# sflorescu/BWA-MEM_GPU

Hardware: AMD Instinct MI355X
Metric: Mreads/s (150 bp single-end vs hg38-scale index; seed-and-extend hot path) (higher is better)
Workload: dtype u16

## Files before the change

bwa-mem_gpu_amd/csrc/seed_kernels.hip:

```cpp
#include <cstring>
#include <string>
#include <vector>
#include <hip/hip_runtime.h>
#include <rocprim/rocprim.hpp>
#include <stdint.h>
#include <stdio.h>
#include <stdlib.h>
#include "bmh_internal.h"
#include "wtrace.h"
#include "fmd_dev.h"
#include "seed_dev.h"


__device__ __forceinline__ int ascii_code(uint8_t ch)
{
	ch &= 0xDF;
	return ch == 'A' ? 0 : ch == 'C' ? 1 : ch == 'G' ? 2 : ch == 'T' ? 3 : 4;
}

#define PACK_READS_PER_BLOCK 64
__global__ void __launch_bounds__(256) pack_reads_kernel(const uint8_t *__restrict__ ascii, const uint32_t *__restrict__ offs,
                                                         const uint32_t *__restrict__ lens, uint32_t n_reads, uint32_t n_grp,
                                                         uint32_t lds_bytes, uint32_t *__restrict__ pk, uint32_t *__restrict__ nm)
{
	wtrace_scope_t wt_(WT_PACK);
	extern __shared__ __attribute__((aligned(16))) uint8_t stage[];
	const uint32_t r0 = blockIdx.x * PACK_READS_PER_BLOCK;
	const uint32_t nr = min((uint32_t)PACK_READS_PER_BLOCK, n_reads - r0);
	const uint32_t first = offs[r0], last = offs[r0 + nr - 1] + lens[r0 + nr - 1];
	const uint32_t abase = first & ~3u;
	const bool staged = last >= first && (last - abase) + 4 <= lds_bytes && (((uintptr_t)ascii) & 3) == 0;
	if (staged) {
		const uint32_t nw = (last - abase + 3) >> 2;
		const uint32_t *src = (const uint32_t *)(ascii + abase);
		for (uint32_t i = threadIdx.x; i < nw; i += blockDim.x) ((uint32_t *)stage)[i] = src[i];
	}
	__syncthreads();
	for (uint32_t it = threadIdx.x; it < nr * n_grp; it += blockDim.x) {
		const uint32_t rr = it % nr, g = it / nr, r = r0 + rr;
		const uint32_t len = lens[r], o = offs[r];
		const bool in_lds = staged && o >= first && o + len <= last;
		const uint8_t *p = in_lds ? stage + (o - abase) : ascii + o;
		uint32_t w0 = 0, w1 = 0, m = 0;
		for (int t = 0; t < 32; ++t) {
			const uint32_t i = g * 32 + t;
			const int c = i < len ? ascii_code(p[i]) : 4;
			if (c > 3) m |= 1u << t;
			else if (t < 16) w0 |= (uint32_t)c << (2 * t);
			else w1 |= (uint32_t)c << (2 * (t - 16));
		}
		pk[(size_t)(2 * g) * n_reads + r] = w0;
		pk[(size_t)(2 * g + 1) * n_reads + r] = w1;
		nm[(size_t)g * n_reads + r] = m;
	}
}


struct cand_t { uint32_t read, xe, j, s; };

#define CAND_CHUNK 1024u
#define CAND_INVALID 0xFFFFFFFFu
// ... 126 lines not shown
		cand_append(want, c, ck, out_a, out_k, counter, cap, cc);
	}
	cand_fill_invalid(cc, out_a, cap);
	if (live) n_cand[r] = j;
	if (iters_out && live) iters_out[r] = it_mine;
	if (fst) {
		if (live) { atomicAdd(fst + 1, (unsigned long long)it_mine); atomicAdd(fst + 8 + (it_mine / 8u < 31u ? it_mine / 8u : 31u), 1ull); }
		if ((threadIdx.x & 63) == 0) { atomicAdd(fst, (unsigned long long)it_wave); atomicAdd(fst + 2, 1ull); atomicMax(fst + 3, (unsigned long long)it_wave); atomicAdd(fst + 40 + (it_wave / 8u < 23u ? it_wave / 8u : 23u), 1ull); }
	}
}


__global__ void __launch_bounds__(256) cand_scatter_kernel(const cand_t *__restrict__ in_a, uint64_t n_list, const uint32_t *__restrict__ cand_base,
                                                           uint32_t *__restrict__ perm)
{
	uint64_t t = (uint64_t)blockIdx.x * blockDim.x + threadIdx.x;
	if (t >= n_list) return;
	const uint2 h = *(const uint2 *)&in_a[t];
	const uint32_t j = in_a[t].j;
	if (h.x == CAND_INVALID) return;
	perm[(size_t)cand_base[h.x] + j] = (uint32_t)t;
}

__global__ void __launch_bounds__(256) iota_kernel(uint32_t *__restrict__ v, uint32_t n) { const uint32_t i = blockIdx.x * 256u + threadIdx.x; if (i < n) v[i] = i; }
#define BWD_NSUB 64
struct bwd_state_t { uint64_t lo, hi; uint32_t read, t; uint16_t x, end, i, beg; };
template <bool RESUME>
__global__ void __launch_bounds__(256) smem_backward_kernel(fmd_dev_t f, read_view_t rv, uint64_t n_cands, int min_seed_len,
                                                            const cand_t *__restrict__ cand_a, const uint64_t *__restrict__ cand_k,
                                                            const uint32_t *__restrict__ perm,
                                                            res_t *__restrict__ res_a, uint64_t *__restrict__ res_k,
                                                            unsigned long long *__restrict__ stats,
                                                            const bwd_state_t *__restrict__ in_state, const uint32_t *__restrict__ in_count,
                                                            bwd_state_t *__restrict__ out_state, uint32_t *__restrict__ out_count, const uint32_t sub_cap, const int max_iter)
{
	wtrace_scope_t wt_(WT_BACKWARD);
	fmd_wave_prio(f.wave_prio);
	uint64_t t = (uint64_t)blockIdx.x * blockDim.x + threadIdx.x;
	const int lane = __lane_id();
	__shared__ uint64_t l2_lds[4];
	if (threadIdx.x < 4) l2_lds[threadIdx.x] = f.L2[threadIdx.x];
	__syncthreads();
	const uint32_t sub = blockIdx.x % BWD_NSUB;
	if (RESUME) {
		n_cands = in_count[sub];
		t = (uint64_t)(blockIdx.x / BWD_NSUB) * blockDim.x + threadIdx.x;
		in_state += (size_t)sub * sub_cap;
		if ((uint64_t)(blockIdx.x / BWD_NSUB) * blockDim.x >= n_cands) return;
	}
	if (out_state) { out_state += (size_t)sub * sub_cap; out_count += sub; }
	bool live = t < n_cands;
	cand_t c = {CAND_INVALID, 0, 0, 0};
	uint64_t lo = 0, hi = 0;
	int x = 0, end = 0, i = -1, beg = 0;
	uint32_t t_out = (uint32_t)t;
	if (RESUME) {
		if (live) { const bwd_state_t s = in_state[t]; lo = s.lo; hi = s.hi; c.read = s.read; t_out = s.t; x = s.x; end = s.end; i = s.i; beg = s.beg; c.s = (uint32_t)(hi - lo + 1); }
	} else {
		if (live) { const uint32_t src = perm[t]; c = cand_a[src]; lo = cand_k[src]; hi = lo + c.s - 1; }
		x = (int)(c.xe >> 16); end = (int)(c.xe & 0xFFFF);
		i = x - 1; beg = x;
	}
	bool act = live && i >= 0, dropped = false;
	const uint32_t nread = __shfl_down(c.read, 1), nx = __shfl_down((uint32_t)x, 1), nt = __shfl_down(t_out, 1);
	const bool last_of_seg = lane == 63 || !live || nread != c.read || nx != (uint32_t)x || nt <= t_out;
	const unsigned long long segb = __ballot(last_of_seg);
	const int seg_end = lane + __builtin_ctzll(segb >> lane);
// ... 13 lines not shown
			const uint64_t L2b = l2_lds[b];
			const uint64_t nl = L2b + ol + 1, nu = L2b + ou;
			const bool ok = !isn && nl <= nu;
			lo = ok ? nl : lo; hi = ok ? nu : hi; beg = ok ? i : beg;
			size = ok ? (uint32_t)(nu - nl + 1) : size;
			i -= ok ? 1 : 0;
			act = ok && i >= 0;
			if (act && (i & 15) == 15) {
				rw = rv.pk[(size_t)(i >> 4) * rv.n_reads + c.read];
				if ((i & 31) == 31) rm = rv.nm[(size_t)(i >> 5) * rv.n_reads + c.read];
			}
		}
		const unsigned long long am = __ballot(act) & above;
		const int nxt = am ? __builtin_ctzll(am) : lane;
		const uint32_t nsize = __shfl(size, nxt);
		if (act && am && nsize == size) { act = false; dropped = true; }
	}
	if (stats) {
		if (live && !RESUME) atomicAdd(stats + 8 + (st_mine < 39u ? st_mine : 39u), 1ull);
		atomicAdd(stats + 1, (unsigned long long)st_steps); atomicAdd(stats + 4, (unsigned long long)st_uniq); atomicAdd(stats + 5, (unsigned long long)st_u0); atomicAdd(stats + 6, (unsigned long long)st_x0); { const bool nowalk = !__any(live && !st_x0); if (!RESUME && lane == 0 && nowalk) atomicAdd(stats + 7, 1ull); }
		if (lane == 0) { atomicAdd(stats, (unsigned long long)st_iter); atomicAdd(stats + 2, 1ull); atomicMax(stats + 3, (unsigned long long)st_iter); }
	}
	const unsigned long long sm = __ballot(act);
	if (sm) {
		const int first = (int)__builtin_ctzll(sm);
		uint32_t base = 0;
		if (lane == first) base = atomicAdd(out_count, (uint32_t)__builtin_popcountll(sm));
		base = __shfl(base, first);
		if (act) {
			bwd_state_t s; s.lo = lo; s.hi = hi; s.read = c.read; s.t = t_out; s.x = (uint16_t)x; s.end = (uint16_t)end; s.i = (uint16_t)i; s.beg = (uint16_t)beg;
			out_state[base + (uint32_t)__builtin_popcountll(sm & ((1ull << lane) - 1ull))] = s;
		}
	}
	if (live && !act) {
		res_t o;
		o.read = c.read; o.be = ((uint32_t)beg << 16) | (uint32_t)end;
		o.s = (!dropped && end - beg >= min_seed_len) ? (uint32_t)(hi - lo + 1) : 0u;
		o.pad = 0;
		res_a[t_out] = o;
		res_k[t_out] = lo;
	}
}


__global__ void __launch_bounds__(256) smem_filter_kernel(const res_t *__restrict__ res_a, uint64_t n, uint32_t *__restrict__ occ)
{
	wtrace_scope_t wt_(WT_FILTER);
	uint64_t t = (uint64_t)blockIdx.x * blockDim.x + threadIdx.x;
	res_t e = {0xFFFFFFFEu, 0, 0, 0};
	if (t < n) e = res_a[t];
	bool k = e.s > 0;
	__shared__ uint32_t fv_has[4], fv_read[4], fv_be[4];
	const int lane = __lane_id(), wv = (int)(threadIdx.x >> 6);
	const unsigned long long vm = __ballot(k);
	if (lane == 0) fv_has[wv] = vm ? 1u : 0u;
	if (vm && lane == (int)__builtin_ctzll(vm)) { fv_read[wv] = e.read; fv_be[wv] = e.be; }
	__syncthreads();
	const unsigned long long ab = lane < 63 ? (vm >> (lane + 1)) << (lane + 1) : 0ull;
	const int nl = ab ? __builtin_ctzll(ab) : lane;
	const uint32_t nread = __shfl(e.read, nl), nbe = __shfl(e.be, nl);
	if (k) {
		if (ab) { if (nread == e.read && (nbe >> 16) == (e.be >> 16)) k = false; }
		else {
			int w2 = wv + 1;
			while (w2 < 4 && !fv_has[w2]) ++w2;
			if (w2 < 4) { if (fv_read[w2] == e.read && (fv_be[w2] >> 16) == (e.be >> 16)) k = false; }
			else {
				for (uint64_t u = (uint64_t)(blockIdx.x + 1) * blockDim.x; u < n; ++u) {
					res_t nx = res_a[u];
					if (nx.read != e.read) break;
					if (nx.s == 0) continue;
					if ((nx.be >> 16) == (e.be >> 16)) k = false;
					break;
				}
			}
		}
	}
	if (t <= n) occ[t] = k ? e.s : 0u;
}

struct occ_keep_in {
	const uint32_t *occ;
	__device__ uint64_t operator()(uint64_t t) const { const uint32_t v = occ[t]; return (uint64_t)v | ((uint64_t)(v != 0u) << OCC_OFF_SHIFT); }
};
__global__ void __launch_bounds__(256) per_read_counts_kernel(const uint32_t *__restrict__ cand_base, const uint64_t *__restrict__ occ_off,
                                                              uint32_t n_reads, uint32_t *__restrict__ n_ref_pos, uint32_t *__restrict__ prefix)
{
	uint32_t r = blockIdx.x * blockDim.x + threadIdx.x;
	if (r >= n_reads) return;
	uint64_t a = occ_off[cand_base[r]] & OCC_OFF_MASK, b = occ_off[cand_base[r + 1]] & OCC_OFF_MASK;
	prefix[r] = (uint32_t)a;
	n_ref_pos[r] = (uint32_t)(b - a);
}


__global__ void __launch_bounds__(256) expand_kernel(const res_t *__restrict__ res_a, const uint64_t *__restrict__ res_k,
                                                     const uint32_t *__restrict__ occ, const uint64_t *__restrict__ occ_off, uint64_t n,
                                                     uint64_t *__restrict__ rows, int2 *__restrict__ qbeg, uint32_t *__restrict__ score)
{
	wtrace_scope_t wt_(WT_EXPAND);
	uint64_t t = (uint64_t)blockIdx.x * blockDim.x + threadIdx.x;
	uint32_t s = 0;
	uint64_t k = 0, off = 0;
	int2 qb = make_int2(0, 0);
	if (t < n) {
		s = occ[t];
		if (s) { res_t e = res_a[t]; k = res_k[t]; off = occ_off[t] & OCC_OFF_MASK; qb = make_int2((int)(e.be >> 16), (int)(e.be & 0xFFFF)); }
	}
	const uint32_t SMALL = 4;
	if (s && s <= SMALL) {
		for (uint32_t u = 0; u < s; ++u) { rows[off + u] = k + u; qbeg[off + u] = qb; score[off + u] = u ? 0u : s; }
// ... 205 lines not shown
	uint64_t t = (uint64_t)blockIdx.x * blockDim.x + threadIdx.x;
	bool v = false;
	if (t < n_list) {
		cand_t c = in_a[t];
		v = c.read != CAND_INVALID;
		keys[t] = v ? (((uint64_t)c.read << 16) | (c.xe & 0xFFFFu)) : ~0ull;
		vals[t] = (uint32_t)t;
	}
	unsigned long long m = __ballot(v);
	if (__lane_id() == 0 && m) atomicAdd(n_valid, (unsigned long long)__popcll(m));
}

__global__ void __launch_bounds__(256) smem_gather_kernel(const cand_t *__restrict__ in_a, const uint64_t *__restrict__ in_k,
                                                          const uint32_t *__restrict__ vals, uint64_t n_valid, res_t *__restrict__ res_a,
                                                          uint64_t *__restrict__ res_k, uint32_t *__restrict__ occ)
{
	uint64_t t = (uint64_t)blockIdx.x * blockDim.x + threadIdx.x;
	if (t > n_valid) return;
	if (t == n_valid) { occ[t] = 0; return; }
	const uint32_t src = vals[t];
	const cand_t c = in_a[src];
	res_t o = {c.read, c.xe, c.s, 0};
	res_a[t] = o;
	res_k[t] = in_k[src];
	occ[t] = c.s;
}


#define HIPCK(x) do { hipError_t e_ = (x); if (e_ != hipSuccess) { bmh_set_error("%s: %s", #x, hipGetErrorString(e_)); return BMH_ENODEV; } } while (0)

struct bmh_seed_ws {
	uint32_t max_reads; uint64_t max_bases, max_cands, max_occ;
	uint32_t *pk, *nm;
	uint32_t n_grp_cap;
	cand_t *cand_a; uint64_t *cand_k;
	res_t *res_a; uint64_t *res_k;
	uint32_t *n_cand, *cand_base;
	uint32_t *occ;
	uint64_t *occ_off;
	uint64_t *rows; int2 *qbeg; uint32_t *score;
	uint32_t *n_ref_pos, *prefix;
	unsigned long long *counter;
	uint4 *scratch; size_t scratch_entries;
	uint64_t *skeys, *skeys2; uint32_t *svals, *svals2;
	bwd_state_t *bwd_state[2]; uint64_t bwd_state_cap;
	uint32_t *bwd_cnt;
	uint32_t *fwd_iters; uint32_t fwd_iters_n;
	void *scan_tmp; size_t scan_tmp_bytes;
	hipEvent_t ev[8];
	float ms[7];
	hipStream_t st_hi; hipEvent_t ev_in, ev_out;
	reseed_state_t *rs;
};

extern "C" bmh_seed_ws_t *bmh_seed_ws_create(uint32_t max_reads, uint64_t max_bases, uint64_t max_cands, uint64_t max_occ)
{
	if (max_reads == 0 || max_bases == 0) { bmh_set_error("bmh_seed_ws_create: empty capacity"); return nullptr; }
	bmh_seed_ws *w = (bmh_seed_ws *)calloc(1, sizeof(bmh_seed_ws));
	w->max_reads = max_reads; w->max_bases = max_bases;
	w->max_cands = max_cands ? max_cands : (uint64_t)max_reads * 16 + max_bases * 2 / 5;
	w->max_cands += ((uint64_t)max_reads / 64 + 1) * (CAND_CHUNK + 64);
	w->max_occ = max_occ ? max_occ : (uint64_t)max_reads * 64;
	w->n_grp_cap = 0;
	bool ok = true;
#define A(p, n) ok = ok && hipMalloc((void **)&(p), (size_t)(n)) == hipSuccess
	A(w->cand_a, sizeof(cand_t) * w->max_cands); A(w->cand_k, 8 * w->max_cands);
	A(w->res_a, sizeof(res_t) * (w->max_cands + 1)); A(w->res_k, 8 * (w->max_cands + 1));
	A(w->n_cand, 4 * ((size_t)max_reads + 1)); A(w->cand_base, 4 * ((size_t)max_reads + 1));
	A(w->occ, 4 * (w->max_cands + 1));
	A(w->occ_off, 8 * (w->max_cands + 1));
	A(w->rows, 8 * w->max_occ); A(w->qbeg, 8 * w->max_occ); A(w->score, 4 * w->max_occ);
	A(w->n_ref_pos, 4 * (size_t)max_reads); A(w->prefix, 4 * (size_t)max_reads);
	A(w->counter, 1024);
	A(w->bwd_cnt, 4 * 8 * BWD_NSUB);
	A(w->skeys, 8 * w->max_cands); A(w->skeys2, 8 * w->max_cands); A(w->svals, 4 * w->max_cands); A(w->svals2, 4 * w->max_cands);
	size_t t1 = 0, t2 = 0, t3 = 0;
	rocprim::radix_sort_pairs(nullptr, t3, w->skeys, w->skeys2, w->svals, w->svals2, (size_t)w->max_cands, 0, 64, 0);
	rocprim::exclusive_scan(nullptr, t1, w->n_cand, w->cand_base, 0u, (size_t)max_reads + 1, rocprim::plus<uint32_t>(), 0);
	rocprim::exclusive_scan(nullptr, t2, w->occ, w->occ_off, (uint64_t)0, w->max_cands + 1, rocprim::plus<uint64_t>(), 0);
	w->scan_tmp_bytes = t1 > t2 ? t1 : t2;
	if (t3 > w->scan_tmp_bytes) w->scan_tmp_bytes = t3;
	A(w->scan_tmp, w->scan_tmp_bytes + 256);
#undef A
	for (int i = 0; i < 8; ++i) ok = ok && hipEventCreate(&w->ev[i]) == hipSuccess;
	{
		const char *pe = getenv("BMH_SEED_PRIO");
		if (!(pe && pe[0] == 'n')) {
			int prio_lo = 0, prio_hi = 0;
			(void)hipDeviceGetStreamPriorityRange(&prio_lo, &prio_hi);
			const char *cue = getenv("BMH_SEED_CUS");
			const int n_cus = cue ? atoi(cue) : 0;
			if (n_cus > 0 && n_cus < 256) {
				uint32_t cumask[8] = {0, 0, 0, 0, 0, 0, 0, 0};
				for (int i = 0; i < n_cus; ++i) { const int b = (i * 167 + 13) & 255; cumask[b >> 5] |= 1u << (b & 31); }
				ok = ok && hipExtStreamCreateWithCUMask(&w->st_hi, 8, cumask) == hipSuccess;
			} else
			ok = ok && hipStreamCreateWithPriority(&w->st_hi, hipStreamNonBlocking, prio_hi) == hipSuccess;
			ok = ok && hipEventCreateWithFlags(&w->ev_in, hipEventDisableTiming) == hipSuccess && hipEventCreateWithFlags(&w->ev_out, hipEventDisableTiming) == hipSuccess;
		}
	}
	if (!ok) { bmh_set_error("bmh_seed_ws_create: hipMalloc failed (%s)", hipGetErrorString(hipGetLastError())); bmh_seed_ws_free(w); return nullptr; }
	return w;
}

extern "C" void bmh_seed_ws_free(bmh_seed_ws_t *w)
{
	if (!w) return;
	void *ps[] = {w->pk, w->nm, w->cand_a, w->cand_k, w->res_a, w->res_k, w->n_cand, w->cand_base, w->occ,
	              w->occ_off, w->rows, w->qbeg, w->score, w->n_ref_pos, w->prefix, w->counter, w->scan_tmp,
	              w->scratch, w->skeys, w->skeys2, w->svals, w->svals2, w->bwd_state[0], w->bwd_state[1], w->bwd_cnt, w->fwd_iters};
	for (void *p : ps) if (p) (void)hipFree(p);
	for (int i = 0; i < 8; ++i) if (w->ev[i]) (void)hipEventDestroy(w->ev[i]);
	if (w->st_hi) (void)hipStreamDestroy(w->st_hi);
	if (w->ev_in) (void)hipEventDestroy(w->ev_in);
	if (w->ev_out) (void)hipEventDestroy(w->ev_out);
	reseed_state_free(w->rs);
	free(w);
}

extern "C" void bmh_seed_last_timing(const bmh_seed_ws_t *w, float ms[7]) { memcpy(ms, w->ms, sizeof(float) * 7); }

static inline unsigned nblk(uint64_t n, unsigned b) { return (unsigned)((n + b - 1) / b); }

static int bwd_state_reserve(bmh_seed_ws *w, uint64_t n)
{
	if (n <= w->bwd_state_cap) return BMH_OK;
	for (int k = 0; k < 2; ++k) { if (w->bwd_state[k]) (void)hipFree(w->bwd_state[k]); w->bwd_state[k] = nullptr; }
	w->bwd_state_cap = 0;
	const uint64_t cap = n + n / 8 + 1024;
	for (int k = 0; k < 2; ++k)
		if (hipMalloc((void **)&w->bwd_state[k], sizeof(bwd_state_t) * cap) != hipSuccess) { bmh_set_error("bmh_seed_batch: no memory for %llu parked walks of the backward search", (unsigned long long)cap); return BMH_ENOMEM; }
	w->bwd_state_cap = cap;
	return BMH_OK;
}

static int grow_occ(bmh_seed_ws *w, uint64_t need, bmh_seeds_t *out)
{
	if (need <= w->max_occ) return BMH_OK;
	(void)hipFree(w->rows); (void)hipFree(w->qbeg); (void)hipFree(w->score);
	w->rows = nullptr; w->qbeg = nullptr; w->score = nullptr; w->max_occ = 0;
	const uint64_t cap = need + need / 4 + 1024;
	if (hipMalloc((void **)&w->rows, 8 * cap) != hipSuccess || hipMalloc((void **)&w->qbeg, 8 * cap) != hipSuccess || hipMalloc((void **)&w->score, 4 * cap) != hipSuccess) {
		bmh_set_error("bmh_seed_batch: %llu occurrences: no memory for the output arrays (%s)", (unsigned long long)need, hipGetErrorString(hipGetLastError()));
		return BMH_ECAPACITY;
	}
	w->max_occ = cap;
	out->d_rbeg = w->rows; out->d_qbeg = (const int32_t *)w->qbeg; out->d_score = w->score;
	return BMH_OK;
}

static int seed_batch_on(bmh_seed_ws_t *w, const bmh_index_t *idx, const uint8_t *d_reads, const uint32_t *d_offs,
                         const uint32_t *d_lens, uint32_t n_reads, int min_seed_len, void *stream_, bmh_seeds_t *out, const bmh_reseed_opt_t *ro = nullptr);
static int seed_batch_impl(bmh_seed_ws_t *w, const bmh_index_t *idx, const uint8_t *d_reads, const uint32_t *d_offs,
                           const uint32_t *d_lens, uint32_t n_reads, int min_seed_len, const bmh_reseed_opt_t *ro, void *stream_, bmh_seeds_t *out);
extern "C" int bmh_seed_batch(bmh_seed_ws_t *w, const bmh_index_t *idx, const uint8_t *d_reads, const uint32_t *d_offs,
                              const uint32_t *d_lens, uint32_t n_reads, int min_seed_len, void *stream_, bmh_seeds_t *out)
{
	return seed_batch_impl(w, idx, d_reads, d_offs, d_lens, n_reads, min_seed_len, nullptr, stream_, out);
}
extern "C" void bmh_reseed_opt_default(bmh_reseed_opt_t *o)
{
	if (!o) return;
	o->enable = 0; o->split_factor = 1.5f; o->split_width = 10; o->max_mem_intv = 20;
}
extern "C" int bmh_seed_batch_reseed(bmh_seed_ws_t *w, const bmh_index_t *idx, const uint8_t *d_reads, const uint32_t *d_offs,
                                     const uint32_t *d_lens, uint32_t n_reads, int min_seed_len, const bmh_reseed_opt_t *opt, void *stream_, bmh_seeds_t *out)
{
	return seed_batch_impl(w, idx, d_reads, d_offs, d_lens, n_reads, min_seed_len, (opt && opt->enable) ? opt : nullptr, stream_, out);
}
static int seed_batch_impl(bmh_seed_ws_t *w, const bmh_index_t *idx, const uint8_t *d_reads, const uint32_t *d_offs,
                           const uint32_t *d_lens, uint32_t n_reads, int min_seed_len, const bmh_reseed_opt_t *ro, void *stream_, bmh_seeds_t *out)
{
	if (!w || !idx || !out) { bmh_set_error("bmh_seed_batch: null argument"); return BMH_EINVAL; }
	if (!w->st_hi) return seed_batch_on(w, idx, d_reads, d_offs, d_lens, n_reads, min_seed_len, stream_, out, ro);
	hipStream_t su = (hipStream_t)stream_;
	HIPCK(hipStreamSynchronize(su));
	const int rc = seed_batch_on(w, idx, d_reads, d_offs, d_lens, n_reads, min_seed_len, (void *)w->st_hi, out, ro);
	HIPCK(hipEventRecord(w->ev_out, w->st_hi));
	HIPCK(hipStreamWaitEvent(su, w->ev_out, 0));
	return rc;
}
static int seed_batch_on(bmh_seed_ws_t *w, const bmh_index_t *idx, const uint8_t *d_reads, const uint32_t *d_offs,
                         const uint32_t *d_lens, uint32_t n_reads, int min_seed_len, void *stream_, bmh_seeds_t *out, const bmh_reseed_opt_t *ro)
{
	memset(out, 0, sizeof(*out));
	if (n_reads > w->max_reads) { bmh_set_error("bmh_seed_batch: %u reads > workspace capacity %u", n_reads, w->max_reads); return BMH_ECAPACITY; }
	if (min_seed_len < 1) { bmh_set_error("bmh_seed_batch: min_seed_len < 1"); return BMH_EINVAL; }
	hipStream_t st = (hipStream_t)stream_;
	out->d_rbeg = w->rows; out->d_qbeg = (const int32_t *)w->qbeg; out->d_score = w->score;
	out->d_n_ref_pos = w->n_ref_pos; out->d_prefix = w->prefix;
	memset(w->ms, 0, sizeof(w->ms));
	if (n_reads == 0) return BMH_OK;
	fmd_dev_t f = idx->dev;
	f.wave_prio = bmh_tune("SEED_SETPRIO", 0);
	const unsigned lds_pad = (unsigned)bmh_tune("SEED_LDS_PAD", 0);
	uint32_t max_len = 0;
	{
		uint32_t *d_max = (uint32_t *)w->counter + 2;
		size_t tb = w->scan_tmp_bytes;
		HIPCK(rocprim::reduce(w->scan_tmp, tb, d_lens, d_max, 0u, (size_t)n_reads, rocprim::maximum<uint32_t>(), st));
		HIPCK(hipMemcpyAsync(&max_len, d_max, 4, hipMemcpyDeviceToHost, st));
		HIPCK(hipStreamSynchronize(st));
	}
	if (max_len > 65535) { bmh_set_error("bmh_seed_batch: read longer than 65535 bases"); return BMH_EINVAL; }
	uint32_t n_grp = (max_len + 31) / 32;
	if (n_grp == 0) n_grp = 1;
	if (n_grp > w->n_grp_cap) {
		if (w->pk) (void)hipFree(w->pk);
		if (w->nm) (void)hipFree(w->nm);
		w->pk = w->nm = nullptr; w->n_grp_cap = 0;
		HIPCK(hipMalloc((void **)&w->pk, (size_t)8 * n_grp * w->max_reads));
		HIPCK(hipMalloc((void **)&w->nm, (size_t)4 * n_grp * w->max_reads));
		w->n_grp_cap = n_grp;
	}
	read_view_t rv = {w->pk, w->nm, n_reads};

	HIPCK(hipEventRecord(w->ev[0], st));
	{
		const uint32_t lds_bytes = PACK_READS_PER_BLOCK * n_grp * 32 + 64;
		pack_reads_kernel<<<nblk(n_reads, PACK_READS_PER_BLOCK), 256, lds_bytes <= 65536 ? lds_bytes : 0, st>>>(d_reads, d_offs, d_lens, n_reads, n_grp, lds_bytes <= 65536 ? lds_bytes : 0, w->pk, w->nm);
	}
	static const bool use_fused = getenv("BMH_SEED_FUSED") != nullptr;
	if (use_fused && !ro) {
		const uint32_t depth = max_len >= (uint32_t)min_seed_len ? max_len - (uint32_t)min_seed_len + 1 : 1;
		static int blocks_per_cu = 0, n_cu = 0;
		if (!blocks_per_cu) {
			int dev = 0; hipDeviceProp_t prop;
			HIPCK(hipGetDevice(&dev)); HIPCK(hipGetDeviceProperties(&prop, dev));
			n_cu = prop.multiProcessorCount;
			HIPCK(hipOccupancyMaxActiveBlocksPerMultiprocessor(&blocks_per_cu, smem_fused_kernel, 256, 0));
			if (blocks_per_cu < 1) blocks_per_cu = 1;
		}
		unsigned grid = (unsigned)(n_cu * blocks_per_cu);
		if (grid > nblk(n_reads, 256)) grid = nblk(n_reads, 256);
		const size_t want = (size_t)depth * grid * 256;
		if (want > w->scratch_entries) {
			if (w->scratch) (void)hipFree(w->scratch);
			w->scratch = nullptr; w->scratch_entries = 0;
			HIPCK(hipMalloc((void **)&w->scratch, want * sizeof(uint4)));
			w->scratch_entries = want;
		}
		HIPCK(hipEventRecord(w->ev[1], st));
		HIPCK(hipMemsetAsync(w->counter, 0, 64, st));
		smem_fused_kernel<<<grid, 256, 0, st>>>(f, rv, d_lens, min_seed_len, w->scratch, w->cand_a, w->cand_k, w->counter,
		                                        w->max_cands, w->n_ref_pos, w->counter + 1, (unsigned int *)(w->counter + 3));
		HIPCK(hipEventRecord(w->ev[2], st));
		unsigned long long cnt[8] = {0};
		HIPCK(hipMemcpyAsync(cnt, w->counter, 64, hipMemcpyDeviceToHost, st));
		HIPCK(hipStreamSynchronize(st));
		const unsigned long long n_list = cnt[0];
		out->n_cands = cnt[1];
		if (getenv("BMH_SEED_STATS")) fprintf(stderr, "[fused] grid %u blocks, waves %llu, wave-iterations %llu (%.0f per wave), rank requests %llu (%.1f per iteration), cands %llu\n", grid, cnt[6], cnt[4], (double)cnt[4] / (double)(cnt[6] ? cnt[6] : 1), cnt[5], (double)cnt[5] / (double)(cnt[4] ? cnt[4] : 1), cnt[1]);
		if (n_list > w->max_cands) { bmh_set_error("bmh_seed_batch: %llu SMEM slots > capacity %llu", n_list, (unsigned long long)w->max_cands); return BMH_ECAPACITY; }
		unsigned long long n_valid = 0;
		if (n_list) {
			smem_key_kernel<<<nblk(n_list, 256), 256, 0, st>>>(w->cand_a, n_list, w->skeys, w->svals, w->counter + 2);
			size_t tb = w->scan_tmp_bytes;
			HIPCK(rocprim::radix_sort_pairs(w->scan_tmp, tb, w->skeys, w->skeys2, w->svals, w->svals2, (size_t)n_list, 0, 64, st));
			HIPCK(hipMemcpyAsync(&n_valid, w->counter + 2, 8, hipMemcpyDeviceToHost, st));
			HIPCK(hipStreamSynchronize(st));
		}
		HIPCK(hipEventRecord(w->ev[3], st));
		smem_gather_kernel<<<nblk(n_valid + 1, 256), 256, 0, st>>>(w->cand_a, w->cand_k, w->svals2, n_valid, w->res_a, w->res_k, w->occ);
		{
			size_t tb = w->scan_tmp_bytes;
			HIPCK(rocprim::exclusive_scan(w->scan_tmp, tb, w->occ, w->occ_off, (uint64_t)0, (size_t)n_valid + 1, rocprim::plus<uint64_t>(), st));
			tb = w->scan_tmp_bytes;
			HIPCK(rocprim::exclusive_scan(w->scan_tmp, tb, w->n_ref_pos, w->prefix, 0u, (size_t)n_reads, rocprim::plus<uint32_t>(), st));
		}
		uint64_t tot = 0;
		HIPCK(hipMemcpyAsync(&tot, w->occ_off + n_valid, 8, hipMemcpyDeviceToHost, st));
		HIPCK(hipStreamSynchronize(st));
		out->n_seeds = tot; out->n_smems = n_valid;
		if (grow_occ(w, tot, out) != BMH_OK) return BMH_ECAPACITY;
		if (tot >> 32) { bmh_set_error("bmh_seed_batch: more than 2^32 occurrences in one batch"); return BMH_ECAPACITY; }
		HIPCK(hipEventRecord(w->ev[4], st));
		if (n_valid)
			expand_kernel<<<nblk(n_valid, 256), 256, 0, st>>>(w->res_a, w->res_k, w->occ, w->occ_off, n_valid, w->rows, w->qbeg, w->score);
		HIPCK(hipEventRecord(w->ev[5], st));
		if (tot)
			locate_kernel<<<nblk(nblk(tot, LOCATE_PER_WAVE) * 64ull, 256), 256, 0, st>>>(f, w->rows, tot);
		HIPCK(hipEventRecord(w->ev[6], st));
		HIPCK(hipStreamSynchronize(st));
		HIPCK(hipGetLastError());
		for (int i = 0; i < 6; ++i) (void)hipEventElapsedTime(&w->ms[i], w->ev[i], w->ev[i + 1]);
		(void)hipEventElapsedTime(&w->ms[6], w->ev[0], w->ev[6]);
		return BMH_OK;
	}
	HIPCK(hipEventRecord(w->ev[1], st));
	HIPCK(hipMemsetAsync(w->counter, 0, 8, st));
	HIPCK(hipMemsetAsync(w->n_cand + n_reads, 0, 4, st));
	{
		static const bool fwd_stats = getenv("BMH_SEED_STATS") != nullptr;
		unsigned long long *d_fst = fwd_stats ? (unsigned long long *)w->counter + 64 : nullptr;
		if (fwd_stats) HIPCK(hipMemsetAsync(d_fst, 0, 64 * 8, st));
		const uint32_t *d_deal = nullptr; uint32_t *d_iters = nullptr;
		if (bmh_tune("SEED_FWD_SORT", 0)) {
			if (!w->fwd_iters) HIPCK(hipMalloc((void **)&w->fwd_iters, 4 * ((size_t)w->max_reads + 1)));
			uint32_t *k0 = (uint32_t *)w->skeys, *k1 = (uint32_t *)w->skeys2;
			if (w->fwd_iters_n == n_reads) {
				iota_kernel<<<nblk(n_reads, 256), 256, 0, st>>>(w->svals, n_reads);
				HIPCK(hipMemcpyAsync(k0, w->fwd_iters, 4 * (size_t)n_reads, hipMemcpyDeviceToDevice, st));
				size_t tb = w->scan_tmp_bytes;
				HIPCK(rocprim::radix_sort_pairs_desc(w->scan_tmp, tb, k0, k1, w->svals, w->svals2, (size_t)n_reads, 0, 32, st));
				d_deal = w->svals2;
			}
			d_iters = w->fwd_iters; w->fwd_iters_n = n_reads;
		}
		smem_forward_kernel<<<nblk(n_reads, 256), 256, lds_pad, st>>>(f, rv, d_lens, min_seed_len, w->cand_a, w->cand_k, w->counter, w->max_cands, w->n_cand, d_fst, d_deal, d_iters);
		if (fwd_stats) {
			unsigned long long h[64];
			HIPCK(hipStreamSynchronize(st));
			HIPCK(hipMemcpy(h, d_fst, sizeof(h), hipMemcpyDeviceToHost));
			fprintf(stderr, "[forward] reads %u, waves %llu, wave-iterations %llu (%.1f per wave, longest %llu), lane-iterations %llu (%.1f per read): lane utilisation %.1f%%\n", n_reads, h[2], h[0],
			        (double)h[0] / (h[2] ? h[2] : 1), h[3], h[1], (double)h[1] / (n_reads ? n_reads : 1), 100.0 * h[1] / (64.0 * (h[0] ? h[0] : 1)));
			fprintf(stderr, "[forward] reads by iterations (0-7, 8-15, .. 248+):"); for (int q = 0; q < 32; ++q) fprintf(stderr, " %llu", h[8 + q]);
			fprintf(stderr, "\n[forward] waves by iterations (0-7, .. 184+):"); for (int q = 0; q < 24; ++q) fprintf(stderr, " %llu", h[40 + q]);
			fprintf(stderr, "\n");
		}
	}
	HIPCK(hipEventRecord(w->ev[2], st));
	{
		size_t tb = w->scan_tmp_bytes;
		HIPCK(rocprim::exclusive_scan(w->scan_tmp, tb, w->n_cand, w->cand_base, 0u, (size_t)n_reads + 1, rocprim::plus<uint32_t>(), st));
	}
	unsigned long long n_list = 0;
	uint32_t n_cands32 = 0;
	HIPCK(hipMemcpyAsync(&n_list, w->counter, 8, hipMemcpyDeviceToHost, st));
	HIPCK(hipMemcpyAsync(&n_cands32, w->cand_base + n_reads, 4, hipMemcpyDeviceToHost, st));
	HIPCK(hipStreamSynchronize(st));
	const unsigned long long n_cands = n_cands32;
	out->n_cands = n_cands;
	if (n_list > w->max_cands) { bmh_set_error("bmh_seed_batch: %llu candidate slots > capacity %llu", n_list, (unsigned long long)w->max_cands); return BMH_ECAPACITY; }
	if (n_list)
		cand_scatter_kernel<<<nblk(n_list, 256), 256, 0, st>>>(w->cand_a, n_list, w->cand_base, w->svals);
	{
		static const bool want_stats = getenv("BMH_SEED_STATS") != nullptr;
		unsigned long long *d_st = want_stats ? (unsigned long long *)w->counter + 8 : nullptr;
		if (want_stats) HIPCK(hipMemsetAsync(d_st, 0, 64 + 40 * 8, st));
		if (n_cands) {
			const std::vector<int> phases = [] {
				std::vector<int> v; const char *e = getenv("BMH_SEED_BWD_PHASES"); std::string t = e ? e : "";
				for (size_t p = 0; p < t.size();) { size_t q = t.find(',', p); if (q == std::string::npos) q = t.size(); const int k = atoi(t.substr(p, q - p).c_str()); if (k > 0) v.push_back(k); p = q + 1; }
				return v; }();
			const int np = (int)(phases.size() < 7 ? phases.size() : 7);
			const unsigned nb = nblk(n_cands, 256);
			const uint32_t sub_cap = ((nb + BWD_NSUB - 1) / BWD_NSUB) * 256u;
			if (np && bwd_state_reserve(w, (uint64_t)sub_cap * BWD_NSUB) != BMH_OK) return BMH_ENOMEM;
			uint32_t *cnt = w->bwd_cnt;
			if (np) HIPCK(hipMemsetAsync(cnt, 0, 4 * (size_t)np * BWD_NSUB, st));
			const int big = 0x7FFFFFFF;
			smem_backward_kernel<false><<<nb, 256, lds_pad, st>>>(f, rv, n_cands, min_seed_len, w->cand_a, w->cand_k, w->svals, w->res_a, w->res_k, d_st,
			                                                nullptr, nullptr, np ? w->bwd_state[0] : nullptr, np ? cnt : nullptr, sub_cap, np ? phases[0] : big);
			for (int ph = 1; ph <= np; ++ph)
				smem_backward_kernel<true><<<(sub_cap / 256u) * BWD_NSUB, 256, 0, st>>>(f, rv, n_cands, min_seed_len, w->cand_a, w->cand_k, w->svals, w->res_a, w->res_k, d_st,
				                                                                       w->bwd_state[(ph - 1) & 1], cnt + (size_t)(ph - 1) * BWD_NSUB, ph < np ? w->bwd_state[ph & 1] : nullptr,
				                                                                       ph < np ? cnt + (size_t)ph * BWD_NSUB : nullptr, sub_cap, ph < np ? phases[ph] : big);
		}
		if (want_stats) {
			unsigned long long h[48];
			HIPCK(hipStreamSynchronize(st));
			HIPCK(hipMemcpy(h, d_st, 64 + 40 * 8, hipMemcpyDeviceToHost));
			fprintf(stderr, "[backward] rank steps per candidate (0, 1, .. 38, 39+):");
			for (int q = 0; q < 40; ++q) fprintf(stderr, " %llu", h[8 + q]);
			fprintf(stderr, "\n");
			fprintf(stderr, "[backward] lane-steps on a one-row interval %llu (%.1f%%), candidates that start on one %llu (%.1f%%)\n", h[4], 100.0 * h[4] / (h[1] ? h[1] : 1), h[5], 100.0 * h[5] / (n_cands ? n_cands : 1));
			fprintf(stderr, "[backward] candidates of a pass that starts at read position 0 (no walk) %llu (%.1f%%); waves made of such only %llu\n", h[6], 100.0 * h[6] / (n_cands ? n_cands : 1), h[7]);
			fprintf(stderr, "[backward] candidates %llu, waves %llu (all phases), wave-iterations %llu (%.1f per wave, max %llu), lane-steps %llu (%.1f per candidate): lane utilisation %.1f%%\n",
			        (unsigned long long)n_cands, h[2], h[0], (double)h[0] / (h[2] ? h[2] : 1), h[3], h[1], (double)h[1] / (n_cands ? n_cands : 1), 100.0 * h[1] / (64.0 * (h[0] ? h[0] : 1)));
		}
	}
	HIPCK(hipEventRecord(w->ev[3], st));
	smem_filter_kernel<<<nblk(n_cands + 1, 256), 256, 0, st>>>(w->res_a, n_cands, w->occ);
	{
		size_t tb = w->scan_tmp_bytes;
		occ_keep_in fin; fin.occ = w->occ;
		HIPCK(rocprim::exclusive_scan(w->scan_tmp, tb, rocprim::make_transform_iterator(rocprim::counting_iterator<uint64_t>(0), fin), w->occ_off, (uint64_t)0,
		                              (size_t)n_cands + 1, rocprim::plus<uint64_t>(), st));
	}
	uint64_t tot[2] = {0, 0};
	HIPCK(hipMemcpyAsync(&tot[0], w->occ_off + n_cands, 8, hipMemcpyDeviceToHost, st));
	HIPCK(hipStreamSynchronize(st));
	tot[1] = tot[0] >> OCC_OFF_SHIFT; tot[0] &= OCC_OFF_MASK;
	if (n_cands >> 28) { bmh_set_error("bmh_seed_batch: more than 2^28 candidates in one batch"); return BMH_ECAPACITY; }
	if (ro) {
		reseed_in_t ri = {f, rv, d_lens, n_reads, max_len, min_seed_len, w->res_a, w->res_k, w->occ, w->occ_off, n_cands, tot[1], *ro, w->n_ref_pos, w->prefix};
		reseed_out_t mo;
		const int rc = reseed_merge(&w->rs, ri, st, &mo);
		if (rc != BMH_OK) return rc;
		out->n_seeds = mo.n_occ; out->n_smems = mo.n;
		if (grow_occ(w, mo.n_occ, out) != BMH_OK) return BMH_ECAPACITY;
		if (mo.n_occ >> 32) { bmh_set_error("bmh_seed_batch_reseed: more than 2^32 occurrences in one batch"); return BMH_ECAPACITY; }
		HIPCK(hipEventRecord(w->ev[4], st));
		if (mo.n)
			expand_kernel<<<nblk(mo.n, 256), 256, 0, st>>>(mo.res_a, mo.res_k, mo.occ, mo.occ_off, mo.n, w->rows, w->qbeg, w->score);
		HIPCK(hipEventRecord(w->ev[5], st));
		if (mo.n_occ)
			locate_kernel<<<nblk(nblk(mo.n_occ, LOCATE_PER_WAVE) * 64ull, 256), 256, lds_pad, st>>>(f, w->rows, mo.n_occ);
		HIPCK(hipEventRecord(w->ev[6], st));
		HIPCK(hipStreamSynchronize(st));
		HIPCK(hipGetLastError());
		for (int i = 0; i < 6; ++i) (void)hipEventElapsedTime(&w->ms[i], w->ev[i], w->ev[i + 1]);
		(void)hipEventElapsedTime(&w->ms[6], w->ev[0], w->ev[6]);
		return BMH_OK;
	}
	out->n_seeds = tot[0]; out->n_smems = tot[1];
// ... 60 lines not shown
```

Before: 41.05.

## Fold read-length max into pack kernel and fuse SMEM filter into backward pass

Removes the separate rocprim max-reduce over read lengths and its blocking host sync. The pack kernel now computes the max length with an atomicMax and writes clamped lengths. Packing is done speculatively with the previous batch's group count and repeated if the batch turns out longer. When no backward phases are configured, the backward kernel applies the within-wave duplicate filter itself, and a small fix-up kernel handles only wave boundaries. This replaces the full filter pass. The costs are extra ballot and shuffle work in the backward kernel and a possible re-run of pack, forward and scan for longer batches.

```diff
diff --git a/bwa-mem_gpu_amd/csrc/seed_kernels.hip b/bwa-mem_gpu_amd/csrc/seed_kernels.hip
--- a/bwa-mem_gpu_amd/csrc/seed_kernels.hip
+++ b/bwa-mem_gpu_amd/csrc/seed_kernels.hip
@@ -21,12 +21,20 @@
 #define PACK_READS_PER_BLOCK 64
 __global__ void __launch_bounds__(256) pack_reads_kernel(const uint8_t *__restrict__ ascii, const uint32_t *__restrict__ offs,
                                                          const uint32_t *__restrict__ lens, uint32_t n_reads, uint32_t n_grp,
-                                                         uint32_t lds_bytes, uint32_t *__restrict__ pk, uint32_t *__restrict__ nm)
+                                                         uint32_t lds_bytes, uint32_t *__restrict__ pk, uint32_t *__restrict__ nm,
+                                                         uint32_t *__restrict__ clen, uint32_t *__restrict__ max_len)
 {
 	wtrace_scope_t wt_(WT_PACK);
 	extern __shared__ __attribute__((aligned(16))) uint8_t stage[];
 	const uint32_t r0 = blockIdx.x * PACK_READS_PER_BLOCK;
 	const uint32_t nr = min((uint32_t)PACK_READS_PER_BLOCK, n_reads - r0);
+	if (clen && threadIdx.x < 64) {
+		const uint32_t len = threadIdx.x < nr ? lens[r0 + threadIdx.x] : 0u;
+		if (threadIdx.x < nr) clen[r0 + threadIdx.x] = min(len, n_grp * 32u);
+		uint32_t m = len;
+		for (int o = 32; o; o >>= 1) m = max(m, (uint32_t)__shfl_xor((int)m, o));
+		if (threadIdx.x == 0 && m > *(volatile uint32_t *)max_len) atomicMax(max_len, m);
+	}
 	const uint32_t first = offs[r0], last = offs[r0 + nr - 1] + lens[r0 + nr - 1];
 	const uint32_t abase = first & ~3u;
 	const bool staged = last >= first && (last - abase) + 4 <= lds_bytes && (((uintptr_t)ascii) & 3) == 0;
@@ -219,7 +227,8 @@
                                                             res_t *__restrict__ res_a, uint64_t *__restrict__ res_k,
                                                             unsigned long long *__restrict__ stats,
                                                             const bwd_state_t *__restrict__ in_state, const uint32_t *__restrict__ in_count,
-                                                            bwd_state_t *__restrict__ out_state, uint32_t *__restrict__ out_count, const uint32_t sub_cap, const int max_iter)
+                                                            bwd_state_t *__restrict__ out_state, uint32_t *__restrict__ out_count, const uint32_t sub_cap, const int max_iter,
+                                                            uint32_t *__restrict__ occ, uint32_t *__restrict__ wave_fix)
 {
 	wtrace_scope_t wt_(WT_BACKWARD);
 	fmd_wave_prio(f.wave_prio);
@@ -299,13 +308,26 @@
 			out_state[base + (uint32_t)__builtin_popcountll(sm & ((1ull << lane) - 1ull))] = s;
 		}
 	}
+	const uint32_t s_out = (!dropped && end - beg >= min_seed_len) ? (uint32_t)(hi - lo + 1) : 0u;
 	if (live && !act) {
 		res_t o;
 		o.read = c.read; o.be = ((uint32_t)beg << 16) | (uint32_t)end;
-		o.s = (!dropped && end - beg >= min_seed_len) ? (uint32_t)(hi - lo + 1) : 0u;
+		o.s = s_out;
 		o.pad = 0;
 		res_a[t_out] = o;
 		res_k[t_out] = lo;
+	}
+	if (!RESUME && occ) {
+		bool k = live && s_out > 0;
+		const unsigned long long vm = __ballot(k);
+		const unsigned long long ab = lane < 63 ? (vm >> (lane + 1)) << (lane + 1) : 0ull;
+		const int nl = ab ? __builtin_ctzll(ab) : lane;
+		const uint32_t nread = __shfl(c.read, nl), nbeg = __shfl((uint32_t)beg, nl);
+		if (k && ab && nread == c.read && nbeg == (uint32_t)beg) k = false;
+		if (live) occ[t] = k ? s_out : 0u;
+		const int lv = vm ? 63 - __builtin_clzll(vm) : 0;
+		const uint32_t lv_read = __shfl(c.read, lv), end_read = __shfl(c.read, 63);
+		if (lane == 0) wave_fix[t >> 6] = (vm && lv_read == end_read) ? (uint32_t)lv + 1u : 0u;
 	}
 }
 
@@ -344,6 +366,26 @@
 		}
 	}
 	if (t <= n) occ[t] = k ? e.s : 0u;
+}
+
+__global__ void __launch_bounds__(256) smem_filter_fix_kernel(const res_t *__restrict__ res_a, uint64_t n, const uint32_t *__restrict__ wave_fix, uint32_t n_waves,
+                                                              uint32_t *__restrict__ occ)
+{
+	wtrace_scope_t wt_(WT_FILTER);
+	const uint32_t w = blockIdx.x * blockDim.x + threadIdx.x;
+	if (w == 0) occ[n] = 0u;
+	if (w >= n_waves) return;
+	const uint32_t fl = wave_fix[w];
+	if (!fl) return;
+	const uint64_t t = (uint64_t)w * 64 + fl - 1;
+	const res_t e = res_a[t];
+	for (uint64_t u = (uint64_t)(w + 1) * 64; u < n; ++u) {
+		const res_t nx = res_a[u];
+		if (nx.read != e.read) break;
+		if (nx.s == 0) continue;
+		if ((nx.be >> 16) == (e.be >> 16)) occ[t] = 0u;
+		break;
+	}
 }
 
 struct occ_keep_in {
@@ -615,7 +657,9 @@
 struct bmh_seed_ws {
 	uint32_t max_reads; uint64_t max_bases, max_cands, max_occ;
 	uint32_t *pk, *nm;
-	uint32_t n_grp_cap;
+	uint32_t n_grp_cap, n_grp_last;
+	uint32_t *clen;
+	uint32_t *wave_fix;
 	cand_t *cand_a; uint64_t *cand_k;
 	res_t *res_a; uint64_t *res_k;
 	uint32_t *n_cand, *cand_base;
@@ -651,6 +695,7 @@
 	A(w->res_a, sizeof(res_t) * (w->max_cands + 1)); A(w->res_k, 8 * (w->max_cands + 1));
 	A(w->n_cand, 4 * ((size_t)max_reads + 1)); A(w->cand_base, 4 * ((size_t)max_reads + 1));
 	A(w->occ, 4 * (w->max_cands + 1));
+	A(w->clen, 4 * (size_t)max_reads); A(w->wave_fix, 4 * (w->max_cands / 64 + 8));
 	A(w->occ_off, 8 * (w->max_cands + 1));
 	A(w->rows, 8 * w->max_occ); A(w->qbeg, 8 * w->max_occ); A(w->score, 4 * w->max_occ);
 	A(w->n_ref_pos, 4 * (size_t)max_reads); A(w->prefix, 4 * (size_t)max_reads);
@@ -689,7 +734,7 @@
 extern "C" void bmh_seed_ws_free(bmh_seed_ws_t *w)
 {
 	if (!w) return;
-	void *ps[] = {w->pk, w->nm, w->cand_a, w->cand_k, w->res_a, w->res_k, w->n_cand, w->cand_base, w->occ,
+	void *ps[] = {w->pk, w->nm, w->clen, w->wave_fix, w->cand_a, w->cand_k, w->res_a, w->res_k, w->n_cand, w->cand_base, w->occ,
 	              w->occ_off, w->rows, w->qbeg, w->score, w->n_ref_pos, w->prefix, w->counter, w->scan_tmp,
 	              w->scratch, w->skeys, w->skeys2, w->svals, w->svals2, w->bwd_state[0], w->bwd_state[1], w->bwd_cnt, w->fwd_iters};
 	for (void *p : ps) if (p) (void)hipFree(p);
@@ -729,6 +774,18 @@
 	}
 	w->max_occ = cap;
 	out->d_rbeg = w->rows; out->d_qbeg = (const int32_t *)w->qbeg; out->d_score = w->score;
+	return BMH_OK;
+}
+
+static int grow_packed(bmh_seed_ws *w, uint32_t n_grp)
+{
+	if (n_grp <= w->n_grp_cap) return BMH_OK;
+	if (w->pk) (void)hipFree(w->pk);
+	if (w->nm) (void)hipFree(w->nm);
+	w->pk = w->nm = nullptr; w->n_grp_cap = 0;
+	HIPCK(hipMalloc((void **)&w->pk, (size_t)8 * n_grp * w->max_reads));
+	HIPCK(hipMalloc((void **)&w->nm, (size_t)4 * n_grp * w->max_reads));
+	w->n_grp_cap = n_grp;
 	return BMH_OK;
 }
 
@@ -777,34 +834,31 @@
 	fmd_dev_t f = idx->dev;
 	f.wave_prio = bmh_tune("SEED_SETPRIO", 0);
 	const unsigned lds_pad = (unsigned)bmh_tune("SEED_LDS_PAD", 0);
+	static const bool use_fused = getenv("BMH_SEED_FUSED") != nullptr;
+	const bool fused = use_fused && !ro;
 	uint32_t max_len = 0;
-	{
+	uint32_t n_grp = w->n_grp_last;
+	if (fused) {
 		uint32_t *d_max = (uint32_t *)w->counter + 2;
 		size_t tb = w->scan_tmp_bytes;
 		HIPCK(rocprim::reduce(w->scan_tmp, tb, d_lens, d_max, 0u, (size_t)n_reads, rocprim::maximum<uint32_t>(), st));
 		HIPCK(hipMemcpyAsync(&max_len, d_max, 4, hipMemcpyDeviceToHost, st));
 		HIPCK(hipStreamSynchronize(st));
-	}
-	if (max_len > 65535) { bmh_set_error("bmh_seed_batch: read longer than 65535 bases"); return BMH_EINVAL; }
-	uint32_t n_grp = (max_len + 31) / 32;
+		if (max_len > 65535) { bmh_set_error("bmh_seed_batch: read longer than 65535 bases"); return BMH_EINVAL; }
+		n_grp = (max_len + 31) / 32;
+	} else if (n_grp == 0) n_grp = (uint32_t)((w->max_bases / w->max_reads + 31) / 32);
 	if (n_grp == 0) n_grp = 1;
-	if (n_grp > w->n_grp_cap) {
-		if (w->pk) (void)hipFree(w->pk);
-		if (w->nm) (void)hipFree(w->nm);
-		w->pk = w->nm = nullptr; w->n_grp_cap = 0;
-		HIPCK(hipMalloc((void **)&w->pk, (size_t)8 * n_grp * w->max_reads));
-		HIPCK(hipMalloc((void **)&w->nm, (size_t)4 * n_grp * w->max_reads));
-		w->n_grp_cap = n_grp;
-	}
+	if (n_grp > 2048) n_grp = 2048;
+	if (grow_packed(w, n_grp) != BMH_OK) return BMH_ENODEV;
 	read_view_t rv = {w->pk, w->nm, n_reads};
+	const auto pack = [&](uint32_t *clen, uint32_t *d_max) {
+		const uint32_t lds_bytes = PACK_READS_PER_BLOCK * n_grp * 32 + 64;
+		pack_reads_kernel<<<nblk(n_reads, PACK_READS_PER_BLOCK), 256, lds_bytes <= 65536 ? lds_bytes : 0, st>>>(d_reads, d_offs, d_lens, n_reads, n_grp, lds_bytes <= 65536 ? lds_bytes : 0, w->pk, w->nm, clen, d_max);
+	};
 
 	HIPCK(hipEventRecord(w->ev[0], st));
-	{
-		const uint32_t lds_bytes = PACK_READS_PER_BLOCK * n_grp * 32 + 64;
-		pack_reads_kernel<<<nblk(n_reads, PACK_READS_PER_BLOCK), 256, lds_bytes <= 65536 ? lds_bytes : 0, st>>>(d_reads, d_offs, d_lens, n_reads, n_grp, lds_bytes <= 65536 ? lds_bytes : 0, w->pk, w->nm);
-	}
-	static const bool use_fused = getenv("BMH_SEED_FUSED") != nullptr;
-	if (use_fused && !ro) {
+	if (fused) {
+		pack(nullptr, nullptr);
 		const uint32_t depth = max_len >= (uint32_t)min_seed_len ? max_len - (uint32_t)min_seed_len + 1 : 1;
 		static int blocks_per_cu = 0, n_cu = 0;
 		if (!blocks_per_cu) {
@@ -870,53 +924,65 @@
 		(void)hipEventElapsedTime(&w->ms[6], w->ev[0], w->ev[6]);
 		return BMH_OK;
 	}
-	HIPCK(hipEventRecord(w->ev[1], st));
-	HIPCK(hipMemsetAsync(w->counter, 0, 8, st));
-	HIPCK(hipMemsetAsync(w->n_cand + n_reads, 0, 4, st));
-	{
-		static const bool fwd_stats = getenv("BMH_SEED_STATS") != nullptr;
-		unsigned long long *d_fst = fwd_stats ? (unsigned long long *)w->counter + 64 : nullptr;
-		if (fwd_stats) HIPCK(hipMemsetAsync(d_fst, 0, 64 * 8, st));
-		const uint32_t *d_deal = nullptr; uint32_t *d_iters = nullptr;
-		if (bmh_tune("SEED_FWD_SORT", 0)) {
-			if (!w->fwd_iters) HIPCK(hipMalloc((void **)&w->fwd_iters, 4 * ((size_t)w->max_reads + 1)));
-			uint32_t *k0 = (uint32_t *)w->skeys, *k1 = (uint32_t *)w->skeys2;
-			if (w->fwd_iters_n == n_reads) {
-				iota_kernel<<<nblk(n_reads, 256), 256, 0, st>>>(w->svals, n_reads);
-				HIPCK(hipMemcpyAsync(k0, w->fwd_iters, 4 * (size_t)n_reads, hipMemcpyDeviceToDevice, st));
-				size_t tb = w->scan_tmp_bytes;
-				HIPCK(rocprim::radix_sort_pairs_desc(w->scan_tmp, tb, k0, k1, w->svals, w->svals2, (size_t)n_reads, 0, 32, st));
-				d_deal = w->svals2;
-			}
-			d_iters = w->fwd_iters; w->fwd_iters_n = n_reads;
-		}
-		smem_forward_kernel<<<nblk(n_reads, 256), 256, lds_pad, st>>>(f, rv, d_lens, min_seed_len, w->cand_a, w->cand_k, w->counter, w->max_cands, w->n_cand, d_fst, d_deal, d_iters);
-		if (fwd_stats) {
-			unsigned long long h[64];
-			HIPCK(hipStreamSynchronize(st));
-			HIPCK(hipMemcpy(h, d_fst, sizeof(h), hipMemcpyDeviceToHost));
-			fprintf(stderr, "[forward] reads %u, waves %llu, wave-iterations %llu (%.1f per wave, longest %llu), lane-iterations %llu (%.1f per read): lane utilisation %.1f%%\n", n_reads, h[2], h[0],
-			        (double)h[0] / (h[2] ? h[2] : 1), h[3], h[1], (double)h[1] / (n_reads ? n_reads : 1), 100.0 * h[1] / (64.0 * (h[0] ? h[0] : 1)));
-			fprintf(stderr, "[forward] reads by iterations (0-7, 8-15, .. 248+):"); for (int q = 0; q < 32; ++q) fprintf(stderr, " %llu", h[8 + q]);
-			fprintf(stderr, "\n[forward] waves by iterations (0-7, .. 184+):"); for (int q = 0; q < 24; ++q) fprintf(stderr, " %llu", h[40 + q]);
-			fprintf(stderr, "\n");
-		}
-	}
-	HIPCK(hipEventRecord(w->ev[2], st));
-	{
-		size_t tb = w->scan_tmp_bytes;
-		HIPCK(rocprim::exclusive_scan(w->scan_tmp, tb, w->n_cand, w->cand_base, 0u, (size_t)n_reads + 1, rocprim::plus<uint32_t>(), st));
-	}
 	unsigned long long n_list = 0;
 	uint32_t n_cands32 = 0;
-	HIPCK(hipMemcpyAsync(&n_list, w->counter, 8, hipMemcpyDeviceToHost, st));
-	HIPCK(hipMemcpyAsync(&n_cands32, w->cand_base + n_reads, 4, hipMemcpyDeviceToHost, st));
-	HIPCK(hipStreamSynchronize(st));
+	for (;;) {
+		HIPCK(hipMemsetAsync(w->counter, 0, 16, st));
+		pack(w->clen, (uint32_t *)w->counter + 2);
+		HIPCK(hipEventRecord(w->ev[1], st));
+		HIPCK(hipMemsetAsync(w->n_cand + n_reads, 0, 4, st));
+		{
+			static const bool fwd_stats = getenv("BMH_SEED_STATS") != nullptr;
+			unsigned long long *d_fst = fwd_stats ? (unsigned long long *)w->counter + 64 : nullptr;
+			if (fwd_stats) HIPCK(hipMemsetAsync(d_fst, 0, 64 * 8, st));
+			const uint32_t *d_deal = nullptr; uint32_t *d_iters = nullptr;
+			if (bmh_tune("SEED_FWD_SORT", 0)) {
+				if (!w->fwd_iters) HIPCK(hipMalloc((void **)&w->fwd_iters, 4 * ((size_t)w->max_reads + 1)));
+				uint32_t *k0 = (uint32_t *)w->skeys, *k1 = (uint32_t *)w->skeys2;
+				if (w->fwd_iters_n == n_reads) {
+					iota_kernel<<<nblk(n_reads, 256), 256, 0, st>>>(w->svals, n_reads);
+					HIPCK(hipMemcpyAsync(k0, w->fwd_iters, 4 * (size_t)n_reads, hipMemcpyDeviceToDevice, st));
+					size_t tb = w->scan_tmp_bytes;
+					HIPCK(rocprim::radix_sort_pairs_desc(w->scan_tmp, tb, k0, k1, w->svals, w->svals2, (size_t)n_reads, 0, 32, st));
+					d_deal = w->svals2;
+				}
+				d_iters = w->fwd_iters; w->fwd_iters_n = n_reads;
+			}
+			smem_forward_kernel<<<nblk(n_reads, 256), 256, lds_pad, st>>>(f, rv, w->clen, min_seed_len, w->cand_a, w->cand_k, w->counter, w->max_cands, w->n_cand, d_fst, d_deal, d_iters);
+			if (fwd_stats) {
+				unsigned long long h[64];
+				HIPCK(hipStreamSynchronize(st));
+				HIPCK(hipMemcpy(h, d_fst, sizeof(h), hipMemcpyDeviceToHost));
+				fprintf(stderr, "[forward] reads %u, waves %llu, wave-iterations %llu (%.1f per wave, longest %llu), lane-iterations %llu (%.1f per read): lane utilisation %.1f%%\n", n_reads, h[2], h[0],
+				        (double)h[0] / (h[2] ? h[2] : 1), h[3], h[1], (double)h[1] / (n_reads ? n_reads : 1), 100.0 * h[1] / (64.0 * (h[0] ? h[0] : 1)));
+				fprintf(stderr, "[forward] reads by iterations (0-7, 8-15, .. 248+):"); for (int q = 0; q < 32; ++q) fprintf(stderr, " %llu", h[8 + q]);
+				fprintf(stderr, "\n[forward] waves by iterations (0-7, .. 184+):"); for (int q = 0; q < 24; ++q) fprintf(stderr, " %llu", h[40 + q]);
+				fprintf(stderr, "\n");
+			}
+		}
+		HIPCK(hipEventRecord(w->ev[2], st));
+		{
+			size_t tb = w->scan_tmp_bytes;
+			HIPCK(rocprim::exclusive_scan(w->scan_tmp, tb, w->n_cand, w->cand_base, 0u, (size_t)n_reads + 1, rocprim::plus<uint32_t>(), st));
+		}
+		unsigned long long cnt_h[2] = {0, 0};
+		HIPCK(hipMemcpyAsync(cnt_h, w->counter, 16, hipMemcpyDeviceToHost, st));
+		HIPCK(hipMemcpyAsync(&n_cands32, w->cand_base + n_reads, 4, hipMemcpyDeviceToHost, st));
+		HIPCK(hipStreamSynchronize(st));
+		n_list = cnt_h[0]; max_len = (uint32_t)cnt_h[1];
+		if (max_len > 65535) { bmh_set_error("bmh_seed_batch: read longer than 65535 bases"); return BMH_EINVAL; }
+		w->n_grp_last = max_len ? (max_len + 31) / 32 : 1;
+		if (w->n_grp_last <= n_grp) break;
+		n_grp = w->n_grp_last;
+		if (grow_packed(w, n_grp) != BMH_OK) return BMH_ENODEV;
+		rv.pk = w->pk; rv.nm = w->nm;
+	}
 	const unsigned long long n_cands = n_cands32;
 	out->n_cands = n_cands;
 	if (n_list > w->max_cands) { bmh_set_error("bmh_seed_batch: %llu candidate slots > capacity %llu", n_list, (unsigned long long)w->max_cands); return BMH_ECAPACITY; }
 	if (n_list)
 		cand_scatter_kernel<<<nblk(n_list, 256), 256, 0, st>>>(w->cand_a, n_list, w->cand_base, w->svals);
+	bool filtered = false;
 	{
 		static const bool want_stats = getenv("BMH_SEED_STATS") != nullptr;
 		unsigned long long *d_st = want_stats ? (unsigned long long *)w->counter + 8 : nullptr;
@@ -934,11 +1000,13 @@
 			if (np) HIPCK(hipMemsetAsync(cnt, 0, 4 * (size_t)np * BWD_NSUB, st));
 			const int big = 0x7FFFFFFF;
 			smem_backward_kernel<false><<<nb, 256, lds_pad, st>>>(f, rv, n_cands, min_seed_len, w->cand_a, w->cand_k, w->svals, w->res_a, w->res_k, d_st,
-			                                                nullptr, nullptr, np ? w->bwd_state[0] : nullptr, np ? cnt : nullptr, sub_cap, np ? phases[0] : big);
+			                                                nullptr, nullptr, np ? w->bwd_state[0] : nullptr, np ? cnt : nullptr, sub_cap, np ? phases[0] : big,
+			                                                np ? nullptr : w->occ, np ? nullptr : w->wave_fix);
+			filtered = np == 0;
 			for (int ph = 1; ph <= np; ++ph)
 				smem_backward_kernel<true><<<(sub_cap / 256u) * BWD_NSUB, 256, 0, st>>>(f, rv, n_cands, min_seed_len, w->cand_a, w->cand_k, w->svals, w->res_a, w->res_k, d_st,
 				                                                                       w->bwd_state[(ph - 1) & 1], cnt + (size_t)(ph - 1) * BWD_NSUB, ph < np ? w->bwd_state[ph & 1] : nullptr,
-				                                                                       ph < np ? cnt + (size_t)ph * BWD_NSUB : nullptr, sub_cap, ph < np ? phases[ph] : big);
+				                                                                       ph < np ? cnt + (size_t)ph * BWD_NSUB : nullptr, sub_cap, ph < np ? phases[ph] : big, nullptr, nullptr);
 		}
 		if (want_stats) {
 			unsigned long long h[48];
@@ -954,7 +1022,8 @@
 		}
 	}
 	HIPCK(hipEventRecord(w->ev[3], st));
-	smem_filter_kernel<<<nblk(n_cands + 1, 256), 256, 0, st>>>(w->res_a, n_cands, w->occ);
+	if (filtered) smem_filter_fix_kernel<<<nblk(nblk(n_cands, 256) * 4ull, 256), 256, 0, st>>>(w->res_a, n_cands, w->wave_fix, nblk(n_cands, 256) * 4u, w->occ);
+	else smem_filter_kernel<<<nblk(n_cands + 1, 256), 256, 0, st>>>(w->res_a, n_cands, w->occ);
 	{
 		size_t tb = w->scan_tmp_bytes;
 		occ_keep_in fin; fin.occ = w->occ;
```

After: 41.33 (median of 6 runs). About the same (+0.7%).
